# fruttasecca/approximated_personalized_pagerank

Measured on AMD Instinct MI355X. Metric: source-nodes/sec grank K=64 L=128 on RMAT-22; 1/2/4/8 MI355X + HBM GB/s, higher is better.
Workload: dtype f64

## Files before the change

approximated_personalized_pagerank_amd/csrc/merge_sv.h:

```cpp
#pragma once
#include "merge_xs.h"

namespace pprk {

constexpr int SV_R = 3;
constexpr int SV_UNIT_LOG = 31;
constexpr int SV_XS = 4;
constexpr size_t SV_LIST_BYTES = (size_t)WAVE * 12;
struct SvGeom {
  int wlog;
  int waves;
  int xt;
  int budget;
  __host__ __device__ constexpr int threads() const { return waves * WAVE; }
  __host__ __device__ constexpr int bm_words() const { return SV_R * (1 << wlog) / 64; }
  __host__ __device__ constexpr size_t sketch_bytes() const { return (size_t)SV_R * ((size_t)1 << wlog) * 4; }
  __host__ __device__ constexpr size_t p2_bytes() const { return (size_t)xt * 20 + (size_t)waves * SV_LIST_BYTES; }
  __host__ __device__ constexpr size_t region() const {
    return sketch_bytes() > p2_bytes() ? sketch_bytes() : p2_bytes();
  }
};
__host__ __device__ constexpr SvGeom sv_geom(int wlog, int waves) {
  return SvGeom{wlog, waves, SV_XS * waves * WAVE, SV_XS * waves * WAVE * 85 / 100 - waves * WAVE};
}
// ... 12 lines not shown
};
__host__ __device__ constexpr size_t x2_bytes(int T) { return (size_t)T * 20; }
__device__ __forceinline__ X2Table x2_carve(unsigned char* p, int T) {
  X2Table t;
  t.keys = reinterpret_cast<uint32_t*>(p);
  t.a = reinterpret_cast<unsigned long long*>(p + (size_t)T * 4);
  t.b = reinterpret_cast<unsigned long long*>(p + (size_t)T * 12);
  t.mask = (uint32_t)T - 1u;
  return t;
}
__device__ __forceinline__ void x2_add(const X2Table& t, int h, unsigned long long lo, uint32_t hi) {
  atomicAdd(&t.a[h], lo & 0xffffffffull);
  atomicAdd(&t.b[h], (lo >> 32) | ((unsigned long long)hi << 32));
}
__device__ __forceinline__ double x2_value(unsigned long long A, unsigned long long B, int F = XS_F) {
  const unsigned long long lo = ((B & 0xffffffffull) << 32) + A;
  const uint32_t hi = (uint32_t)(B >> 32) + (lo < A ? 1u : 0u);
  return xs_to_double(hi, lo, F);
}
__device__ __forceinline__ int x2_find(const X2Table& t, int key) {
  const uint32_t tag = (uint32_t)key + 1u;
  uint32_t g = hash32((uint32_t)key) & t.mask & ~3u;
  for (uint32_t n = 0; n <= t.mask; n += 4) {
    const uint4 q = *reinterpret_cast<const uint4*>(t.keys + g);
    const int m = xt_match(q, g, tag);
    if (m >= 0) return m;
    if (q.x == 0u || q.y == 0u || q.z == 0u || q.w == 0u) return -1;
    g = (g + 4u) & t.mask;
  }
  return -1;
}
__device__ __forceinline__ int x2_slot(const X2Table& t, int key, bool& ins) {
  const uint32_t tag = (uint32_t)key + 1u;
  uint32_t g = hash32((uint32_t)key) & t.mask & ~3u;
  ins = false;
  const uint32_t groups = (t.mask + 1u) >> 2;
  uint32_t moves = 0, races = 0;
  while (moves < groups && races <= groups) {
    const uint4 q = *reinterpret_cast<const uint4*>(t.keys + g);
    const int m = xt_match(q, g, tag);
    if (m >= 0) return m;
    const int e = q.x == 0u ? 0 : q.y == 0u ? 1 : q.z == 0u ? 2 : q.w == 0u ? 3 : -1;
    if (e >= 0) {
      const uint32_t prev = atomicCAS(&t.keys[g + e], 0u, tag);
      if (prev == 0u) { ins = true; return (int)(g + e); }
      if (prev == tag) return (int)(g + e);
      races++;
      continue;
    }
    g = (g + 4u) & t.mask;
    moves++;
  }
  return -1;
}

struct SvHash {
  uint32_t h0, h1, h2;
};
__device__ __forceinline__ SvHash sv_hash(int key) {
  const uint32_t k = (uint32_t)key;
  return SvHash{k * 0x9E3779B1u, k * 0x85EBCA77u, k * 0xC2B2AE3Du};
}
__device__ __forceinline__ uint32_t sv_units31(double p31) { return (uint32_t)p31 + 1u; }
__device__ __forceinline__ uint32_t sv_units(double p) { return sv_units31(p * 0x1p31); }
__device__ __forceinline__ uint32_t sv_thr(double theta) {
  const double x = floor(ldexp(theta, SV_UNIT_LOG) * (1.0 - 0x1p-40));
  return x <= 0.0 ? 0u : x >= 4294967295.0 ? 0xffffffffu : (uint32_t)x;
}
__device__ __forceinline__ void sv_sketch_add(uint32_t* sk, const SvHash& hs, uint32_t u, int wlog) {
  const int sh = 32 - wlog;
  atomicAdd(&sk[hs.h0 >> sh], u);
  atomicAdd(&sk[(1u << wlog) + (hs.h1 >> sh)], u);
  atomicAdd(&sk[(2u << wlog) + (hs.h2 >> sh)], u);
}
__device__ __forceinline__ bool sv_passes(const uint32_t* bm, const SvHash& hs, int wlog) {
  const int sh = 32 - wlog;
  const int rw = (1 << wlog) >> 5;
  const uint32_t w0 = bm[hs.h0 >> (sh + 5)];
  const uint32_t w1 = bm[rw + (hs.h1 >> (sh + 5))];
  const uint32_t w2 = bm[2 * rw + (hs.h2 >> (sh + 5))];
  return ((w0 >> ((hs.h0 >> sh) & 31u)) & (w1 >> ((hs.h1 >> sh) & 31u)) & (w2 >> ((hs.h2 >> sh) & 31u)) & 1u) != 0u;
}
__device__ __forceinline__ void sv_split_t(double t, unsigned long long& A, unsigned long long& B) {
  const uint32_t bh = (uint32_t)(t * 0x1p-32);
  const uint32_t bl = (uint32_t)fma(-(double)bh, 0x1p32, t);
  A = (unsigned long long)(uint32_t)(__builtin_amdgcn_fract(t) * 0x1p32);
  B = ((unsigned long long)bh << 32) | bl;
}
__device__ __forceinline__ void sv_split_add_t(unsigned long long* ab, int i, double t) {
  unsigned long long A, B;
  sv_split_t(t, A, B);
  atomicAdd(&ab[2 * i], A);
  atomicAdd(&ab[2 * i + 1], B);
}
__device__ __forceinline__ void sv_split_add(unsigned long long* ab, int i, double p) {
  sv_split_add_t(ab, i, p * 0x1p61);
}
__device__ __forceinline__ void sv_split_add_t(unsigned long long* a, unsigned long long* b, int i, double t) {
  unsigned long long A, B;
  sv_split_t(t, A, B);
  atomicAdd(&a[i], A);
  atomicAdd(&b[i], B);
}
__device__ __forceinline__ void sv_split_add(unsigned long long* a, unsigned long long* b, int i, double p) {
  sv_split_add_t(a, b, i, p * 0x1p61);
}

struct SvPt {
  uint32_t* keys;
  unsigned long long* ab;
  int* pos;
  int T;
  uint32_t gmask;
};
__host__ __device__ constexpr size_t svpt_bytes(int Lp) { return (size_t)4 * Lp * 24 + 64 * 16; }
__device__ __forceinline__ SvPt svpt_carve(unsigned char* p, int Lp) {
  SvPt t;
  t.T = 4 * Lp;
  t.ab = reinterpret_cast<unsigned long long*>(p); p += (size_t)(t.T + 64) * 16;
  t.keys = reinterpret_cast<uint32_t*>(p); p += (size_t)t.T * 4;
  t.pos = reinterpret_cast<int*>(p);
  t.gmask = (uint32_t)(t.T / 4) - 1u;
  return t;
}
constexpr uint32_t SV_OVF_BIT = 0x80000000u;
__device__ __forceinline__ uint32_t svpt_home(const SvPt& t, uint32_t h0) { return __umulhi(h0, (uint32_t)t.T) & ~3u; }
__device__ __forceinline__ int svpt_find_from(const SvPt& t, uint32_t tag, uint32_t g4) {
  for (int n = 0; n < (int)t.gmask + 1; n++) {
    g4 = (g4 + 4u) & (uint32_t)(t.T - 1);
    const uint4 q = *reinterpret_cast<const uint4*>(t.keys + g4);
    const uint32_t x = q.x & ~SV_OVF_BIT;
    if (x == tag) return (int)g4;
    if (q.y == tag) return (int)g4 + 1;
    if (q.z == tag) return (int)g4 + 2;
    if (q.w == tag) return (int)g4 + 3;
    if (x == 0u || q.y == 0u || q.z == 0u || q.w == 0u) return -1;
  }
  return -1;
}
__device__ __forceinline__ int svpt_slot(const SvPt& t, int key, uint32_t h, bool active) {
  const uint32_t tag = (uint32_t)key + 1u;
  const uint32_t g4 = svpt_home(t, h);
  const uint4 q = *reinterpret_cast<const uint4*>(t.keys + g4);
  int m = q.w == tag ? 3 : -1;
  m = q.z == tag ? 2 : m;
  m = q.y == tag ? 1 : m;
  m = (q.x & ~SV_OVF_BIT) == tag ? 0 : m;
  int slot = m >= 0 ? (int)g4 + m : -1;
  const bool more = active && m < 0 && (q.x & SV_OVF_BIT);
  if (__builtin_expect(__ballot(more) != 0ull, 0)) {
    if (more) slot = svpt_find_from(t, tag, g4);
  }
  return slot;
}

struct SvDesc {
  int32_t v;
  int32_t S;
  double factor;
  int64_t gsk;
  int64_t gpt;
  int64_t gxt;
  int32_t tg;
  int32_t pad;
};
struct SvTask { int32_t d; int32_t k; };

enum { SVM_FILL = 0, SVM_OVF = 1, SVM_U = 2, SVM_PT = 3, SVM_ROWS = 4, SVM_THETA = 8  };
__host__ __device__ constexpr size_t sv_lds_bytes(int Lp, SvGeom G) {
  return G.region() + svpt_bytes(Lp) + (size_t)G.bm_words() * 8 + 256 + 1024;
}
struct SvLds {
  unsigned char* region;
  SvPt pt;
  uint64_t* bm;
  int* misc;
  uint32_t* hist;
  int wlog;
  int bm_words;
};
__device__ __forceinline__ SvLds sv_carve(unsigned char* smem, int Lp, SvGeom G) {
  SvLds x;
  unsigned char* p = smem;
  x.region = p; p += G.region();
  x.pt = svpt_carve(p, Lp); p += svpt_bytes(Lp);
  x.bm = reinterpret_cast<uint64_t*>(p); p += (size_t)G.bm_words() * 8;
  x.misc = reinterpret_cast<int*>(p); p += 256;
  x.hist = reinterpret_cast<uint32_t*>(p);
  x.wlog = G.wlog;
  x.bm_words = G.bm_words();
  return x;
}

__device__ __forceinline__ void sv_lap(const IterArgs& a, int slot, long long& t) {
  if (!a.diag || threadIdx.x != 0) return;
  const long long now = (long long)clock64();
  diag_add(a.diag, slot, (unsigned long long)(now - t));
  t = now;
}

template <class KeyAt>
__device__ __forceinline__ void sv_build_pt_keys(const SvLds& x, int n, KeyAt keyat) {
  const SvPt& t = x.pt;
  for (int i = threadIdx.x; i < t.T; i += blockDim.x) t.keys[i] = 0u;
  for (int i = threadIdx.x; i < 2 * (t.T + 64); i += blockDim.x) t.ab[i] = 0ull;
  if (threadIdx.x < 64) x.misc[threadIdx.x] = 0;
  __syncthreads();
  for (int i = threadIdx.x; i < n; i += blockDim.x) {
    const int key = keyat(i);
    const uint32_t tag = (uint32_t)key + 1u;
    const uint32_t home = svpt_home(t, sv_hash(key).h0);
    uint32_t g4 = home;
    for (int n = 0; n <= (int)t.gmask; n++) {
      int got = -1;
#pragma unroll
      for (int j = 0; j < 4 && got < 0; j++)
        if (atomicCAS(&t.keys[g4 + j], 0u, tag) == 0u) got = (int)g4 + j;
      if (got >= 0) { t.pos[got] = i; break; }
      if (g4 == home) atomicOr(&t.keys[home], SV_OVF_BIT);
      g4 = (g4 + 4u) & (uint32_t)(t.T - 1);
    }
  }
}
__device__ __forceinline__ void sv_build_pt(const SvLds& x, const DevSlab& s, const IterArgs& a, int v, int Lp,
                                            const int32_t* seeds = nullptr) {
  const int cur = (a.active == 1) ? a.sB : a.sA;
  const int64_t r = s.row(cur, v);
  const int n = seeds ? s.L : s.len[s.lrow(cur, v)];
  sv_build_pt_keys(x, n, [&](int i) { return seeds ? (int)seeds[i] : s.key(s.ids[r + i]); });
}

template <int NS>
struct SvBatch {
  int key[2 * NS];
  double sv[2 * NS];
  int rl[NS];
  int64_t base[NS];
};
template <int NS, class G>
__device__ __forceinline__ void sv_groups(const SvBatch<NS>& bt, G g) {
  const int lane = lane_id();
#pragma unroll
  for (int k = 0; k < 2 * NS; k++) {
    const int rl = bt.rl[k >> 1];
    if ((k & 1) && rl <= WAVE) continue;
    g(k, bt.key[k], bt.sv[k], (k & 1) * WAVE + lane < rl, bt.base[k >> 1] + (k & 1) * WAVE + lane);
  }
}
__device__ __forceinline__ int64_t sv_readlane64(int64_t x, int lane) {
  const uint32_t lo = (uint32_t)__builtin_amdgcn_readlane((int)(uint32_t)x, lane);
  const uint32_t hi = (uint32_t)__builtin_amdgcn_readlane((int)(uint32_t)((uint64_t)x >> 32), lane);
  return (int64_t)(((uint64_t)hi << 32) | lo);
}
template <bool kScores, int NS, class FB, class RM = WalkNoSucc>
__device__ __forceinline__ void sv_rows(const DevGraph& g, const DevSlab& s, const IterArgs& a, int64_t c0, int64_t c1,
                                        FB fb, RM succ = RM{}) {
  const int lane = lane_id();
  const int lcl = lane < s.L ? lane : 0;
  const int lhi = WAVE + lane < s.L ? WAVE + lane : lcl;
  auto colx_at = [&](int64_t w0) { return w0 + lane < c1 ? g.colx[w0 + lane] : (int32_t)-1; };
  auto len_of = [&](int32_t cx) { return cx == -1 ? 0 : s.len[s.lrow(read_slot(a, cx), cx & 0x7fffffff)]; };
  auto base_of = [&](int32_t cx) { return cx == -1 ? (int64_t)0 : s.row(read_slot(a, cx), cx & 0x7fffffff); };
  auto rmin_of = [&](int32_t cx) {
    return cx == -1 ? 0ull : dbits(s.rmin[s.lrow(read_slot(a, cx), cx & 0x7fffffff)]);
  };
  int32_t ncx = colx_at(c0);
  int32_t nncx = c0 + WAVE < c1 ? colx_at(c0 + WAVE) : -1;
  int nln = len_of(ncx);
  unsigned long long nrm = RM::kWant ? rmin_of(ncx) : 0ull;
  for (int64_t w0 = c0; w0 < c1; w0 += WAVE) {
    const int32_t cx = ncx;
    const int ln = nln;
    if (RM::kWant) succ(ln, nrm);
    const int64_t base = base_of(cx);
    ncx = nncx;
    if (w0 + 2 * WAVE < c1) nncx = colx_at(w0 + 2 * WAVE);
    nln = len_of(ncx);
    if (RM::kWant) nrm = rmin_of(ncx);
    const int nrows = (int)min((int64_t)WAVE, c1 - w0);
    auto load = [&](int q0, SvBatch<NS>& bt) {
#pragma unroll
      for (int q = 0; q < NS; q++) {
        const bool has = q0 + q < nrows;
        const int qq = has ? q0 + q : 0;
        bt.rl[q] = has ? __builtin_amdgcn_readlane(ln, qq) : 0;
        bt.base[q] = has ? sv_readlane64(base, qq) : (int64_t)0;
        bt.key[2 * q] = s.ids[bt.base[q] + lcl];
        if (kScores) bt.sv[2 * q] = s.sc[bt.base[q] + lcl];
        const int i2 = bt.rl[q] > WAVE ? lhi : lcl;
        bt.key[2 * q + 1] = s.ids[bt.base[q] + i2];
        if (kScores) bt.sv[2 * q + 1] = s.sc[bt.base[q] + i2];
      }
    };
    auto run = [&](const SvBatch<NS>& bt) { fb(bt); };
    SvBatch<NS> ba, bb;
    load(0, ba);
    for (int q0 = 0; q0 < nrows; q0 += 2 * NS) {
      load(q0 + NS, bb);
      __builtin_amdgcn_sched_barrier(0);
      run(ba);
      __builtin_amdgcn_sched_barrier(0);
      if (q0 + NS >= nrows) break;
      load(q0 + 2 * NS, ba);
      __builtin_amdgcn_sched_barrier(0);
      run(bb);
      __builtin_amdgcn_sched_barrier(0);
    }
  }
}

__device__ __forceinline__ int64_t sv_uniform(int64_t x) {
  const uint32_t lo = (uint32_t)__builtin_amdgcn_readfirstlane((int)(uint32_t)x);
  const uint32_t hi = (uint32_t)__builtin_amdgcn_readfirstlane((int)(uint32_t)((uint64_t)x >> 32));
  return (int64_t)(((uint64_t)hi << 32) | lo);
}
__device__ __forceinline__ void sv_chunk(int64_t b0, int64_t b1, int64_t& c0, int64_t& c1) {
  const int W = blockDim.x >> 6, wv = threadIdx.x >> 6;
  const int64_t chunk = (b1 - b0 + W - 1) / W;
  c0 = sv_uniform(b0 + (int64_t)wv * chunk);
  c1 = sv_uniform(min(b1, c0 + chunk));
}

#ifndef PPR_SV_NS1
#define PPR_SV_NS1 4
#endif
#ifndef PPR_SV_NS2
#define PPR_SV_NS2 4
#endif
#ifndef PPR_SV_P2_SCORES
#define PPR_SV_P2_SCORES 0
#endif
constexpr bool SV_P2_SCORES = PPR_SV_P2_SCORES != 0;
#ifndef PPR_SV_WALK_ONLY
#define PPR_SV_WALK_ONLY 0
#endif
#ifndef PPR_SV_NO_INSERT
#define PPR_SV_NO_INSERT 0
#endif
constexpr int SV_NS1 = PPR_SV_NS1, SV_NS2 = PPR_SV_NS2;
__device__ __forceinline__ void sv_pass1(const DevGraph& g, const DevSlab& s, const IterArgs& a, const SvLds& x,
                                         int64_t b0, int64_t b1, double factor, uint32_t* sk) {
  int64_t c0, c1;
  sv_chunk(b0, b1, c0, c1);
  const double f61 = factor * 0x1p61, f31 = factor * 0x1p31;
  sv_rows<true, SV_NS1>(g, s, a, c0, c1, [&](const SvBatch<SV_NS1>& bt) {
    sv_groups(bt, [&](int, int key, double sc, bool valid, int64_t) {
      const SvHash hs = sv_hash(key);
      const int slot = svpt_slot(x.pt, key, hs.h0, valid);
      const bool inpt = valid && slot >= 0;
      if (inpt) sv_split_add_t(x.pt.ab, slot, sc * f61);
      if (valid && !inpt) sv_sketch_add(sk, hs, sv_units31(sc * f31), x.wlog);
    });
  });
}

#ifndef PPR_SV_LIST
#define PPR_SV_LIST 1
#endif
__device__ __forceinline__ void sv_insert(const SvLds& x, const X2Table& xt, const IterArgs& a, bool live, int key,
                                          double t, int budget, bool keep) {
  const int lane = lane_id();
  const bool w = live && svpt_slot(x.pt, key, sv_hash(key).h0, live) < 0;
  if (!__ballot(w)) return;
  if (a.diag && lane == 0) diag_add(a.diag, 148, 1ull);
  if (__hip_atomic_load(&x.misc[SVM_FILL], __ATOMIC_RELAXED, __HIP_MEMORY_SCOPE_WORKGROUP) > budget) {
    if (lane == 0) x.misc[SVM_OVF] = 1;
    if (keep) {
      const int hs = w ? x2_find(xt, key) : -1;
      if (hs >= 0) sv_split_add_t(xt.a, xt.b, hs, t);
    }
    return;
  }
  bool ins = false;
  int hs = -1;
  if (w) hs = x2_slot(xt, key, ins);
  const int nins = __popcll(__ballot(ins));
  if (nins && lane == 0) atomicAdd(&x.misc[SVM_FILL], nins);
  if (__ballot(w && hs < 0) && lane == 0) x.misc[SVM_OVF] = 1;
  if (hs >= 0) sv_split_add_t(xt.a, xt.b, hs, t);
  if (a.diag && lane == 0) diag_add(a.diag, 138, (unsigned long long)__popcll(__ballot(w)));
}
__device__ __forceinline__ void sv_pass2(const DevGraph& g, const DevSlab& s, const IterArgs& a, const SvLds& x,
                                         const X2Table& xt, int64_t b0, int64_t b1, double factor, int budget,
                                         bool keep = false) {
  int64_t c0, c1;
  sv_chunk(b0, b1, c0, c1);
  const uint32_t* bm32 = reinterpret_cast<const uint32_t*>(x.bm);
  const double f61 = factor * 0x1p61;
  const int lane = lane_id();
  const uint64_t lt = lanemask_lt();
  double* lst = reinterpret_cast<double*>(x.region + (size_t)(xt.mask + 1u) * 20 + (size_t)(threadIdx.x >> 6) * SV_LIST_BYTES);
  int* lsk = reinterpret_cast<int*>(lst + WAVE);
// ... 620 lines not shown
```

approximated_personalized_pagerank_amd/csrc/merge_xs.h:

```cpp
#pragma once
#include "merge_hub.h"
#include "xs_table.h"

namespace pprk {

constexpr double XR_SPEC = 0.9;

__host__ __device__ constexpr size_t lds_wave_bytes_x(int T, int Lp) {
  return (size_t)T * 16 + (size_t)Lp * 12 + 1024 + (size_t)Lp * 20;
}
__host__ __device__ constexpr size_t lds_wave_bytes_xs(int T) { return (size_t)T * 16 + 1024; }


#ifndef PPR_WX_WAVES
#define PPR_WX_WAVES 1
#endif
template <bool kSplit>
__global__ void __launch_bounds__(256, kSplit ? PPR_WX_WAVES : 1) k_merge_lds_x(DevGraph g, DevSlab s, IterArgs a, const int32_t* list,
                                                     int64_t count, int T, int Lp, unsigned long long* maxdiff,
                                                     unsigned long long* stats, int32_t* dlast, int32_t* wovl,
                                                     WList wl) {
  extern __shared__ __align__(16) unsigned char smem[];
  const int wv = threadIdx.x >> 6;
  const int64_t w = (int64_t)blockIdx.x * (blockDim.x >> 6) + wv;
  if (w >= count) return;
  unsigned char* base = smem + (size_t)wv * (kSplit ? lds_wave_bytes_xs(T) : lds_wave_bytes_x(T, Lp));
  const XTable t = xt_carve(base, T);
  uint32_t* hist = reinterpret_cast<uint32_t*>(base + (size_t)T * 16);
  uint64_t* rv = reinterpret_cast<uint64_t*>(base + (size_t)T * 16 + 1024);
  int* rk = reinterpret_cast<int*>(base + (size_t)T * 16 + 1024 + (size_t)Lp * 8);
  int* hk = reinterpret_cast<int*>(base + (size_t)T * 16 + 1024 + (size_t)Lp * 12);
  int* hv = hk + 2 * Lp;
  int* mf = hv + 2 * Lp;

  const int v = list[w];
  const int64_t b = g.rp[v], e = g.rp[v + 1];
  const double factor = merge_factor(a, e - b);
  long long tl = a.diag ? (long long)clock64() : 0;
  for (int i = lane_id(); i < T; i += WAVE) { t.keys[i] = 0u; t.lo[i] = 0ull; t.hi[i] = 0u; }
  wave_fence();
  bool bad = false;
  if (lane_id() == 0) {
    unsigned long long lo;
    uint32_t hi;
    xs_conv(self_seed(a, e - b), lo, hi, a.xsf);
    bad = xt_add(t, v, lo, hi) < 0;
  }
  wave_fence();
  unsigned long long mb = 0;
  if (a.unit) {
    unsigned long long flo;
    uint32_t fhi;
    xs_conv(factor, flo, fhi, a.xsf);
    for (int64_t e0 = b; e0 < e; e0 += WAVE) {
      const int64_t i = e0 + lane_id();
      if (i < e && xt_add(t, g.colx[i] & 0x7fffffff, flo, fhi) < 0) bad = true;
    }
  } else {
    for (int64_t e0 = b; e0 < e; e0 += WAVE)
      hub_window_walk(g, s, a, e0, min(e, e0 + WAVE), reinterpret_cast<uint8_t*>(hist),
                      [&](bool valid, int id, double sv, bool) {
                        if (valid) {
                          unsigned long long lo;
                          uint32_t hi;
                          xs_conv(sv * factor, lo, hi, a.xsf);
                          if (xt_add(t, id, lo, hi) < 0) bad = true;
                        }
                      },
                      WalkRowMin{&mb, (int)s.L});
  }
  wave_fence();
  if (__ballot(bad)) {
    if (lane_id() == 0) {
      wovl[1 + atomicAdd(&wovl[0], 1)] = v;
      if (kSplit) wl.n[w] = -1;
    }
    return;
  }
  fs_lap(a, 280, 1, tl);
#pragma unroll
  for (int o = 32; o; o >>= 1) { const unsigned long long y = __shfl_xor(mb, o); mb = y > mb ? y : mb; }
  const double tau = (!a.unit && mb) ? xs_single(bitsd(mb) * factor, a.xsf) : 0.0;
  double* vals = reinterpret_cast<double*>(t.lo);
  int* keys = reinterpret_cast<int*>(t.keys);
  double tspec = 0.0;
  if (!a.unit && !a.mc) {
    const int64_t cr = s.lrow((a.active == 1) ? a.sB : a.sA, v);
    if (s.len[cr] == s.L) tspec = fmax(tau, XR_SPEC * s.rmin[cr]);
  }
  int U = 0, D = 0, Uhi = 0;
  for (int base0 = 0; base0 < T; base0 += WAVE) {
    const int i = base0 + lane_id();
    const uint32_t kt = t.keys[i];
    const unsigned long long lo = t.lo[i];
    const bool occ = kt != 0u;
    const double x = occ ? xs_to_double(t.hi[i], lo, a.xsf) : 0.0;
    const bool keep = occ && x >= tau;
    const uint64_t m = __ballot(keep);
    D += __popcll(__ballot(occ));
    Uhi += __popcll(__ballot(keep && x >= tspec));
    wave_fence();
    if (keep) {
      const int pos = U + __popcll(m & lanemask_lt());
      vals[pos] = x;
      keys[pos] = (int)kt - 1;
    }
    wave_fence();
    U += __popcll(m);
  }
  if (tspec > tau && Uhi >= (int)s.L && Uhi < U) {
    int U2 = 0;
    for (int i0 = 0; i0 < U; i0 += WAVE) {
      const int i = i0 + lane_id();
      const double x = i < U ? vals[i] : 0.0;
      const int k = i < U ? keys[i] : 0;
      const bool keep = i < U && x >= tspec;
      const uint64_t m = __ballot(keep);
      wave_fence();
      if (keep) { const int pos = U2 + __popcll(m & lanemask_lt()); vals[pos] = x; keys[pos] = k; }
      wave_fence();
      U2 += __popcll(m);
    }
    U = U2;
  }
  if (dlast && !a.unit && lane_id() == 0) dlast[v] = D;
  fs_lap(a, 280, 2, tl);
  if (a.diag && !a.unit && lane_id() == 0) { diag_add(a.diag, 280, 1ull); diag_add(a.diag, 287, (unsigned long long)U); }
  if (kSplit) {
    wave_emit_list(wl, w, U, keys, vals, v, (int)s.L, hist);
  } else {
    finish_source(v, U, [&](int i) { return keys[i]; }, [&](int i) { return vals[i]; }, s, a, hist, rv, rk, Lp, hk, hv,
                  mf, maxdiff, stats, a.unit ? -1 : 283);
  }
}

__host__ __device__ constexpr size_t wfin_lds_bytes(int Lp) { return (size_t)Lp * 12 + 1024 + (size_t)Lp * 20; }
__global__ void __launch_bounds__(256) k_wfin(DevSlab s, IterArgs a, const int32_t* list, int64_t count, WList wl,
                                              int Lp, unsigned long long* maxdiff, unsigned long long* stats) {
  extern __shared__ __align__(16) unsigned char smem[];
  const int wv = threadIdx.x >> 6;
  const int64_t w = (int64_t)blockIdx.x * (blockDim.x >> 6) + wv;
  if (w >= count) return;
  const int n = wl.n[w];
  if (n < 0) return;
  unsigned char* base = smem + (size_t)wv * wfin_lds_bytes(Lp);
  uint64_t* rv = reinterpret_cast<uint64_t*>(base);
  int* rk = reinterpret_cast<int*>(base + (size_t)Lp * 8);
  uint32_t* hist = reinterpret_cast<uint32_t*>(base + (size_t)Lp * 12);
  int* hk = reinterpret_cast<int*>(base + (size_t)Lp * 12 + 1024);
  int* hv = hk + 2 * Lp;
  int* mf = hv + 2 * Lp;
  const int64_t o = w * (int64_t)wl.cap;
  const int32_t* lk = wl.k + o;
  const double* lv = wl.v + o;
  finish_source(list[w], n, [&](int i) { return lk[i]; }, [&](int i) { return lv[i]; }, s, a, hist, rv, rk, Lp, hk,
                hv, mf, maxdiff, stats, 283);
}

__host__ __device__ constexpr size_t xr_lds_bytes(int T, int W, int Lp) {
  return (size_t)T * 16 + (size_t)W * HUB_WALK_FLAGS + 1024 + 256 + (size_t)Lp * 32;
}

struct XDesc {
  int32_t v;
  int32_t R;
  int64_t pt_off;
  double factor, selfval;
};

enum { XM_FILL = 0, XM_OVF = 1, XM_CNT = 2, XM_U = 3, XM_MIN = 10  };

struct XrLds {
  XTable t;
  uint8_t* fl;
  WgLds w;
};

__device__ __forceinline__ XrLds xr_carve(unsigned char* smem, int T, int W, int Lp) {
  XrLds x;
  unsigned char* p = smem;
  x.t = xt_carve(p, T); p += xt_bytes(T);
  x.fl = p; p += (size_t)W * HUB_WALK_FLAGS;
  x.w = WgLds{};
  x.w.hist = reinterpret_cast<uint32_t*>(p); p += 1024;
  x.w.misc = reinterpret_cast<int*>(p); p += 256;
  x.w.rv = reinterpret_cast<uint64_t*>(p); p += (size_t)Lp * 8;
  x.w.rk = reinterpret_cast<int*>(p); p += (size_t)Lp * 4;
  x.w.hk = reinterpret_cast<int*>(p); p += (size_t)Lp * 8;
  x.w.hv = reinterpret_cast<int*>(p); p += (size_t)Lp * 8;
  x.w.mf = reinterpret_cast<int*>(p);
  return x;
}

__device__ __forceinline__ void xr_lap(const IterArgs& a, int slot, long long& t) {
  if (!a.diag || threadIdx.x != 0) return;
  const long long now = (long long)clock64();
  diag_add(a.diag, slot, (unsigned long long)(now - t));
  t = now;
}

__device__ __forceinline__ void xr_clear(const XrLds& x, int T) {
  for (int i = threadIdx.x; i < T; i += blockDim.x) { x.t.keys[i] = 0u; x.t.lo[i] = 0ull; x.t.hi[i] = 0u; }
  if (threadIdx.x < 64) x.w.misc[threadIdx.x] = 0;
}

constexpr int XR_FULL = 1 << 24;
__device__ __forceinline__ void xr_apply(const XrLds& x, bool valid, int key, double p, int budget, int F) {
  int r = 0;
  if (valid) {
    unsigned long long lo;
    uint32_t hi;
    xs_conv(p, lo, hi, F);
    r = xt_add(x.t, key, lo, hi);
  }
  const int n = __popcll(__ballot(r > 0)) + (__ballot(r < 0) ? XR_FULL : 0);
  if (n && lane_id() == 0) atomicAdd(&x.w.misc[XM_FILL], n);
}
__device__ __forceinline__ bool xr_stop(const XrLds& x, int budget) {
  return __hip_atomic_load(&x.w.misc[XM_FILL], __ATOMIC_RELAXED, __HIP_MEMORY_SCOPE_WORKGROUP) > budget;
}

constexpr int XR_SLOTS = 8;
__device__ __forceinline__ void xr_finish(const XrLds& x, int T, const DevSlab& s, const IterArgs& a,
                                          const XDesc& xd, int d, bool publish, double tau0, double tau_spec,
                                          unsigned long long* xtau, int32_t* pk, double* ps, uint32_t* pc,
                                          uint32_t* dsum, long long* tph = nullptr, int slot = 0, int cap = 0) {
  const int L = s.L;
  const int v = xd.v;
  if (publish) tau0 = fmax(tau0, bitsd(__hip_atomic_load(&xtau[d], __ATOMIC_RELAXED, __HIP_MEMORY_SCOPE_AGENT)));
  const double ts_hi = fmax(tau0, tau_spec);
  int kk[XR_SLOTS];
  double kv[XR_SLOTS];
  int c = 0, c_hi = 0;
  uint32_t kt[XR_SLOTS], kh[XR_SLOTS];
  unsigned long long kl[XR_SLOTS];
#pragma unroll
  for (int j = 0; j < XR_SLOTS; j++) {
    const int i = min(T - 1, (int)threadIdx.x + j * (int)blockDim.x);
    kt[j] = x.t.keys[i];
    kl[j] = x.t.lo[i];
    kh[j] = x.t.hi[i];
  }
#pragma unroll
  for (int j = 0; j < XR_SLOTS; j++) {
    const bool in = (int)threadIdx.x + j * (int)blockDim.x < T;
    kv[j] = xs_to_double(kh[j], kl[j], a.xsf);
    kk[j] = (in && kt[j] && kv[j] >= tau0) ? (int)kt[j] - 1 : -1;
    c += kk[j] >= 0 ? 1 : 0;
    c_hi += (kk[j] >= 0 && kv[j] >= ts_hi) ? 1 : 0;
  }
  if (tau_spec > tau0) {
    const int w_hi = wave_sum(c_hi);
    if (lane_id() == 0 && w_hi) atomicAdd(&x.w.misc[XM_CNT], w_hi);
    __syncthreads();
    if (x.w.misc[XM_CNT] >= L) {
      tau0 = ts_hi;
      c = c_hi;
#pragma unroll
      for (int j = 0; j < XR_SLOTS; j++)
        if (kk[j] >= 0 && kv[j] < ts_hi) kk[j] = -1;
    }
  }
  const int incl = wave_incl_scan(c);
  int base = 0;
  if (lane_id() == WAVE - 1 && incl) base = atomicAdd(&x.w.misc[XM_U], incl);
  base = __builtin_amdgcn_readlane(base, WAVE - 1) + incl - c;
  __syncthreads();
  int* dk = reinterpret_cast<int*>(x.t.keys);
  double* dv = reinterpret_cast<double*>(x.t.lo);
#pragma unroll
  for (int j = 0; j < XR_SLOTS; j++)
    if (kk[j] >= 0) { dk[base] = kk[j]; dv[base] = kv[j]; base++; }
  __syncthreads();
  const int D = x.w.misc[XM_FILL];
  const int U = x.w.misc[XM_U];
  if (threadIdx.x == 0 && D) atomicAdd(&dsum[d], (uint32_t)D);
  const uint32_t ts = tie_salt(v);
  auto keyat = [&](int i) { return dk[i]; };
  auto valat = [&](int i) { return dv[i]; };
  SelCrit sc;
  sc.tie = false; sc.pa = 0; sc.ma = 0; sc.pb = 0; sc.mb = 0;
  const bool cut = U > L && !(cap && !publish && U <= cap);
  if (tph) xr_lap(a, slot, *tph);
  if (cut) sc = wg_select_top(x.w, U, L, keyat, valat, [](int) { return true; }, ts);
  if (tph) xr_lap(a, slot + 1, *tph);
  double tb = tau0;
  if (publish) {
    if (cut) {
      unsigned long long* wmin = reinterpret_cast<unsigned long long*>(&x.w.misc[XM_MIN]);
      if (threadIdx.x == 0) *wmin = ~0ull;
      __syncthreads();
      unsigned long long mn = ~0ull;
      for (int i = threadIdx.x; i < U; i += blockDim.x) {
        const unsigned long long vb = dbits(dv[i]);
        if (sel_test(sc, vb, tie_w(dk[i], ts))) mn = vb < mn ? vb : mn;
      }
      mn = wave_min_u64(mn);
      if (lane_id() == 0 && mn != ~0ull) atomicMin(wmin, mn);
      __syncthreads();
      if (threadIdx.x == 0 && *wmin != ~0ull) atomicMax(&xtau[d], *wmin);
      __syncthreads();
    }
    tb = fmax(tb, bitsd(__hip_atomic_load(&xtau[d], __ATOMIC_RELAXED, __HIP_MEMORY_SCOPE_AGENT)));
  }
  for (int i0 = 0; i0 < U; i0 += blockDim.x) {
    const int i = i0 + threadIdx.x;
    bool k = false;
    if (i < U) {
      const uint64_t vb = dbits(dv[i]);
      k = dv[i] >= tb && (!cut || sel_test(sc, vb, tie_w(dk[i], ts)));
    }
    const uint64_t m = __ballot(k);
    uint32_t b0 = 0;
    if (m && lane_id() == 0) b0 = atomicAdd(&pc[d], (uint32_t)__popcll(m));
    b0 = (uint32_t)__shfl((int)b0, 0);
    if (k) {
      const int64_t o = xd.pt_off + b0 + __popcll(m & lanemask_lt());
      pk[o] = dk[i];
      ps[o] = dv[i];
    }
  }
  if (tph) xr_lap(a, slot + 2, *tph);
}

__host__ __device__ constexpr size_t xf1_lds_bytes(int Lp) { return (size_t)Lp * 12 + 1024 + (size_t)Lp * 20; }
__global__ void __launch_bounds__(64) k_xfin1(DevSlab s, IterArgs a, const XDesc* xdesc, int d0, const int32_t* pk,
                                              const double* ps, const uint32_t* pc, const uint32_t* dsum,
                                              const int32_t* skip, int32_t* dlast, int Lp,
                                              unsigned long long* maxdiff, unsigned long long* stats) {
  extern __shared__ __align__(16) unsigned char smem[];
  const int d = d0 + (int)blockIdx.x;
  if (skip[d]) return;
  const XDesc xd = xdesc[d];
  uint64_t* rv = reinterpret_cast<uint64_t*>(smem);
  int* rk = reinterpret_cast<int*>(smem + (size_t)Lp * 8);
  uint32_t* hist = reinterpret_cast<uint32_t*>(smem + (size_t)Lp * 12);
  int* hk = reinterpret_cast<int*>(smem + (size_t)Lp * 12 + 1024);
  int* hv = hk + 2 * Lp;
  int* mf = hv + 2 * Lp;
  const int n = (int)pc[d];
  if (dlast && !a.unit && lane_id() == 0) dlast[xd.v] = (int32_t)dsum[d];
  const int32_t* lk = pk + xd.pt_off;
  const double* lv = ps + xd.pt_off;
  finish_source(xd.v, n, [&](int i) { return lk[i]; }, [&](int i) { return lv[i]; }, s, a, hist, rv, rk, Lp, hk, hv, mf,
                maxdiff, stats);
}

__device__ __forceinline__ bool xr_in(int key, int r, int R) {
  return R == 1 || (int)(((uint64_t)hash_b((uint32_t)key) * (uint32_t)R) >> 32) == r;
}

struct XTask { int32_t d; int32_t r; };

__global__ void __launch_bounds__(1024) k_xr(DevGraph g, DevSlab s, IterArgs a, const XDesc* xdesc,
                                             const XTask* tasks, int T, int budget, int Lp, unsigned long long* xtau,
                                             int32_t* pk, double* ps, uint32_t* pc, uint32_t* dsum,
                                             int32_t* oflag, int32_t* ovl, int xcap) {
  extern __shared__ __align__(16) unsigned char smem[];
  const int W = blockDim.x >> 6, wv = threadIdx.x >> 6;
  const XrLds x = xr_carve(smem, T, W, Lp);
  const XTask tk = tasks[blockIdx.x];
  const XDesc xd = xdesc[tk.d];
  const int v = xd.v, R = xd.R, r = tk.r;
  long long tph = a.diag ? (long long)clock64() : 0;
  xr_clear(x, T);
  __syncthreads();
  if (threadIdx.x == 0 && xr_in(v, r, R)) {
    unsigned long long lo;
    uint32_t hi;
    xs_conv(xd.selfval, lo, hi, a.xsf);
    xt_add(x.t, v, lo, hi);
    x.w.misc[XM_FILL] = 1;
  }
  __syncthreads();
  xr_lap(a, 183, tph);
  const int64_t b = g.rp[v], e = g.rp[v + 1];
  const double factor = xd.factor;
  unsigned long long mb = 0;
  uint8_t* fl = x.fl + (size_t)wv * HUB_WALK_FLAGS;
  auto fn = [&](bool valid, int id, double sv, bool) {
#if defined(PPR_XR_WALK_ONLY)
    if (valid && id == -9 && sv == -1.0) x.w.misc[XM_FILL] = 1;
    return;
#endif
    if (xr_stop(x, budget)) return;
    xr_apply(x, valid && xr_in(id, r, R), id, sv * factor, budget, a.xsf);
  };
  if (a.unit) {
    for (int64_t e0 = b + (int64_t)wv * WAVE; e0 < e; e0 += (int64_t)W * WAVE) {
      const int64_t i = e0 + lane_id();
      const int key = i < e ? (g.colx[i] & 0x7fffffff) : 0;
      if (xr_stop(x, budget)) break;
      xr_apply(x, i < e && xr_in(key, r, R), key, factor, budget, a.xsf);
    }
  } else {
    const int64_t chunk = (e - b + W - 1) / W;
    const int64_t c0 = b + (int64_t)wv * chunk, c1 = min(e, c0 + chunk);
    for (int64_t w0 = c0; w0 < c1; w0 += WAVE)
      hub_window_walk(g, s, a, w0, min(c1, w0 + WAVE), fl, fn, WalkRowMin{&mb, (int)s.L});
  }
  __syncthreads();
  xr_lap(a, 184, tph);
  if (a.diag && threadIdx.x == 0) {
    diag_add(a.diag, 182, 1ull);
    diag_add(a.diag, 188, (unsigned long long)(xd.R > 0 ? (e - b) : 0));
    diag_add(a.diag, 189, (unsigned long long)x.w.misc[XM_FILL]);
  }
  if (x.w.misc[XM_FILL] > budget) {
    if (threadIdx.x == 0 && atomicExch(&oflag[tk.d], 1) == 0) ovl[1 + atomicAdd(&ovl[0], 1)] = tk.d;
    return;
  }
#pragma unroll
  for (int o = 32; o; o >>= 1) { const unsigned long long y = __shfl_xor(mb, o); mb = y > mb ? y : mb; }
  if (lane_id() == 0 && mb) atomicMax(reinterpret_cast<unsigned long long*>(&x.w.misc[8]), mb);
  __syncthreads();
  const unsigned long long mbb = *reinterpret_cast<unsigned long long*>(&x.w.misc[8]);
  const double tau_rows = (!a.unit && mbb) ? xs_single(bitsd(mbb) * factor, a.xsf) : 0.0;
  double tau_spec = 0.0;
  if (R == 1 && !a.unit && !a.mc) {
    const int64_t cr = s.lrow((a.active == 1) ? a.sB : a.sA, v);
    if (s.len[cr] == s.L) tau_spec = XR_SPEC * s.rmin[cr];
  }
  xr_finish(x, T, s, a, xd, tk.d, R > 1, tau_rows, tau_spec, xtau, pk, ps, pc, dsum, a.diag ? &tph : nullptr, 185, xcap);
}

constexpr int XB_BATCH = 4;
__global__ void __launch_bounds__(1024) k_xb(DevSlab s, IterArgs a, const HubDesc* desc, const HubTask* tasks,
                                             const int32_t* cm, const uint32_t* staged, const HubRec* st,
                                             const unsigned long long* tau_b, int T, int budget, int Lp,
                                             unsigned long long* xtau, int32_t* pk, double* ps, uint32_t* pc,
                                             uint32_t* dsum, int32_t* oflag, int32_t* ovl, const int64_t* rp) {
  extern __shared__ __align__(16) unsigned char smem[];
  const int W = blockDim.x >> 6, wv = threadIdx.x >> 6;
  const XrLds x = xr_carve(smem, T, W, Lp);
  const HubTask tk = tasks[blockIdx.x];
  const HubDesc d = desc[tk.d];
  int64_t start, nb;
  hub_bucket_range(d, cm, staged[tk.d], tk.x, start, nb);
  const int v = d.v;
  const int64_t deg = rp[v + 1] - rp[v];
  const double factor = merge_factor(a, deg);
  long long tph = a.diag ? (long long)clock64() : 0;
  xr_clear(x, T);
  __syncthreads();
  if (threadIdx.x == 0 && (int)hub_digit(v, d.logP) == tk.x) {
    unsigned long long lo;
    uint32_t hi;
    xs_conv(self_seed(a, deg), lo, hi, a.xsf);
    xt_add(x.t, v, lo, hi);
    x.w.misc[XM_FILL] = 1;
  }
  __syncthreads();
  const HubRec* rec = st + start;
  const int64_t ng = (nb + WAVE - 1) / WAVE;
  struct Batch { HubRec r[XB_BATCH]; };
  auto load = [&](int64_t g0, Batch& hr) {
#pragma unroll
    for (int k = 0; k < XB_BATCH; k++) {
      const int64_t q = (g0 + (int64_t)k * W) * WAVE + lane_id();
      hr.r[k] = rec[q < nb ? q : nb - 1];
    }
  };
  int hk = -1;
  unsigned long long hlo = 0ull;
  uint32_t hhi = 0u;
  auto apply = [&](int64_t g0, const Batch& hr) {
    bool v[XB_BATCH];
    int key[XB_BATCH];
    unsigned long long lo[XB_BATCH];
    uint32_t hi[XB_BATCH], g[XB_BATCH];
    uint4 q[XB_BATCH];
#pragma unroll
    for (int k = 0; k < XB_BATCH; k++) {
      const int64_t gk = g0 + (int64_t)k * W;
      key[k] = rec_key(hr.r[k]);
      v[k] = gk < ng && gk * WAVE + lane_id() < nb;
      xs_conv(rec_sc(hr.r[k]) * factor, lo[k], hi[k], a.xsf);
      if (v[k] && key[k] == hk) {
        const unsigned long long nl = hlo + lo[k];
        hhi += hi[k] + (nl < hlo ? 1u : 0u);
        hlo = nl;
        v[k] = false;
      }
      g[k] = hash32((uint32_t)key[k]) & x.t.mask & ~3u;
    }
#pragma unroll
    for (int k = 0; k < XB_BATCH; k++) q[k] = *reinterpret_cast<const uint4*>(x.t.keys + g[k]);
    int h[XB_BATCH];
#pragma unroll
    for (int k = 0; k < XB_BATCH; k++) {
      h[k] = xt_match(q[k], g[k], (uint32_t)key[k] + 1u);
      if (__ballot(v[k] && h[k] < 0)) {
        if (xr_stop(x, budget)) {
          if (h[k] < 0) v[k] = false;
        } else {
          bool ins = false;
          if (v[k] && h[k] < 0) h[k] = xt_slot(x.t, key[k], ins);
          const bool full = v[k] && h[k] < 0;
          if (full) v[k] = false;
          const int nins = __popcll(__ballot(ins)) + (__ballot(full) ? XR_FULL : 0);
          if (nins && lane_id() == 0) atomicAdd(&x.w.misc[XM_FILL], nins);
        }
      }
    }
    unsigned long long old[XB_BATCH];
#pragma unroll
    for (int k = 0; k < XB_BATCH; k++) {
      if (!v[k]) { h[k] = 0; lo[k] = 0ull; hi[k] = 0u; }
      old[k] = atomicAdd(&x.t.lo[h[k]], lo[k]);
    }
#pragma unroll
    for (int k = 0; k < XB_BATCH; k++) atomicAdd(&x.t.hi[h[k]], hi[k] + ((old[k] + lo[k] < old[k]) ? 1u : 0u));
  };
  Batch ba, bb;
  const int64_t step = (int64_t)W * XB_BATCH;
  if (wv < ng) {
    load(wv, ba);
    const bool v0 = (int64_t)wv * WAVE + lane_id() < nb;
    const int k0 = rec_key(ba.r[0]);
    int best = 0;
#pragma unroll
    for (int c = 0; c < 8; c++) {
      const int cand = __builtin_amdgcn_readlane(k0, c * 8);
      const int n = __popcll(__ballot(v0 && k0 == cand));
      if (n > best && __builtin_amdgcn_readlane((int)v0, c * 8)) { best = n; hk = cand; }
    }
    if (best < 8) hk = -1;
  }
  for (int64_t g0 = wv; g0 < ng; g0 += 2 * step) {
    load(g0 + step < ng ? g0 + step : g0, bb);
    __builtin_amdgcn_sched_barrier(0);
    apply(g0, ba);
    __builtin_amdgcn_sched_barrier(0);
    if (g0 + step >= ng) break;
    load(g0 + 2 * step < ng ? g0 + 2 * step : g0, ba);
    __builtin_amdgcn_sched_barrier(0);
    apply(g0 + step, bb);
    __builtin_amdgcn_sched_barrier(0);
  }
  if (hk >= 0 && (hlo | hhi)) {
    const int r = xt_add(x.t, hk, hlo, hhi);
    if (r) atomicAdd(&x.w.misc[XM_FILL], r > 0 ? 1 : XR_FULL);
  }
  __syncthreads();
  xr_lap(a, 155, tph);
  if (a.diag && threadIdx.x == 0) {
    diag_add(a.diag, 154, 1ull);
    diag_add(a.diag, 159, (unsigned long long)nb);
  }
  if (x.w.misc[XM_FILL] > budget) {
    if (threadIdx.x == 0 && atomicExch(&oflag[tk.d], 1) == 0) ovl[1 + atomicAdd(&ovl[0], 1)] = v;
    return;
  }
  const double tau_rows = (!a.unit && tau_b[tk.d]) ? xs_single(bitsd(tau_b[tk.d]) * factor, a.xsf) : 0.0;
  XDesc xd;
  xd.v = v; xd.R = 0; xd.pt_off = d.pt_off; xd.factor = factor; xd.selfval = 0.0;
  xr_finish(x, T, s, a, xd, tk.d, true, tau_rows, 0.0, xtau, pk, ps, pc, dsum, a.diag ? &tph : nullptr, 156);
}

constexpr int XF_STAGE = 4096;
// ... 74 lines not shown
```

approximated_personalized_pagerank_amd/csrc/xs_table.h:

```cpp
#pragma once
#include "ppr_common.h"

namespace pprk {

__device__ __forceinline__ void xs_conv(double p, unsigned long long& lo, uint32_t& hi, int F = XS_F) {
  const unsigned long long b = dbits(p);
  int e = (int)((b >> 52) & 0x7ffu);
  unsigned long long m = b & ((1ull << 52) - 1ull);
  if (e) m |= 1ull << 52; else e = 1;
  const int sh = e - 1075 + F;
  if (sh >= 0) {
    lo = m << sh;
    hi = sh > 11 ? (uint32_t)(m >> (64 - sh)) : 0u;
  } else {
    lo = -sh < 64 ? (m >> -sh) : 0ull;
    hi = 0u;
  }
}

__device__ __forceinline__ double xs_to_double(uint32_t hi, unsigned long long lo, int F = XS_F) {
  if (hi == 0u) return ldexp((double)lo, -F);
  const int n = 32 - __clz(hi);
  const unsigned long long top = ((unsigned long long)hi << (64 - n)) | (lo >> n);
  const unsigned long long sticky = (lo & ((1ull << n) - 1ull)) != 0ull ? 1ull : 0ull;
  return ldexp((double)(top | sticky), n - F);
}

__device__ __forceinline__ double xs_single(double p, int F = XS_F) {
  unsigned long long lo;
  uint32_t hi;
  xs_conv(p, lo, hi, F);
  return xs_to_double(hi, lo, F);
}

struct XTable {
  uint32_t* keys;
  unsigned long long* lo;
  uint32_t* hi;
  uint32_t mask;
};

__device__ __forceinline__ int xt_add(const XTable& t, int key, unsigned long long xlo, uint32_t xhi) {
  const uint32_t tag = (uint32_t)key + 1u;
  uint32_t g = hash32((uint32_t)key) & t.mask & ~3u;
  int ins = 0;
  uint32_t h = 0;
  const uint32_t groups = (t.mask + 1u) >> 2;
  uint32_t moves = 0, races = 0;
  for (;;) {
    if (moves >= groups || races > groups) return -1;
    const uint4 q = *reinterpret_cast<const uint4*>(t.keys + g);
    if (q.x == tag) { h = g; break; }
    if (q.y == tag) { h = g + 1; break; }
    if (q.z == tag) { h = g + 2; break; }
    if (q.w == tag) { h = g + 3; break; }
    const int e = q.x == 0u ? 0 : q.y == 0u ? 1 : q.z == 0u ? 2 : q.w == 0u ? 3 : -1;
    if (e >= 0) {
      const uint32_t prev = atomicCAS(&t.keys[g + e], 0u, tag);
      if (prev == 0u) { h = g + e; ins = 1; break; }
      if (prev == tag) { h = g + e; break; }
      races++;
      continue;
    }
    g = (g + 4u) & t.mask;
    moves++;
  }
  const unsigned long long old = atomicAdd(&t.lo[h], xlo);
  const uint32_t up = xhi + ((old + xlo < old) ? 1u : 0u);
  if (up) atomicAdd(&t.hi[h], up);
  return ins;
}

__device__ __forceinline__ int xt_match(const uint4& q, uint32_t g, uint32_t tag) {
  return q.x == tag ? (int)g : q.y == tag ? (int)g + 1 : q.z == tag ? (int)g + 2 : q.w == tag ? (int)g + 3 : -1;
}
__device__ __forceinline__ int xt_slot(const XTable& t, int key, bool& ins) {
  const uint32_t tag = (uint32_t)key + 1u;
  uint32_t g = hash32((uint32_t)key) & t.mask & ~3u;
  ins = false;
  const uint32_t groups = (t.mask + 1u) >> 2;
  uint32_t moves = 0, races = 0;
  while (moves < groups && races <= groups) {
    const uint4 q = *reinterpret_cast<const uint4*>(t.keys + g);
    const int m = xt_match(q, g, tag);
    if (m >= 0) return m;
    const int e = q.x == 0u ? 0 : q.y == 0u ? 1 : q.z == 0u ? 2 : q.w == 0u ? 3 : -1;
    if (e >= 0) {
      const uint32_t prev = atomicCAS(&t.keys[g + e], 0u, tag);
      if (prev == 0u) { ins = true; return (int)(g + e); }
      if (prev == tag) return (int)(g + e);
      races++;
      continue;
    }
    g = (g + 4u) & t.mask;
    moves++;
  }
  return -1;
}

__host__ __device__ constexpr size_t xt_bytes(int T) { return (size_t)T * 16; }
// ... 11 lines not shown
```

Before: 3.977 million.

## Use FP-arithmetic fixed-point conversion and batched row walk in LDS merge

Replaces the bit-manipulation double-to-fixed-point conversion (exponent/mantissa shifts with branches) with a branch-free floating-point split into three 32-bit words, and pre-multiplies the scale into the factor once per row. It also moves the batched, software-pipelined row walker into a shared header and uses it in the LDS merge kernel for short rows (L <= 128) in place of the per-window hub walk. The FP-based conversion truncates instead of shifting mantissa bits, which can change rounding or behaviour for very large or very small values.

```diff
diff --git a/approximated_personalized_pagerank_amd/csrc/merge_sv.h b/approximated_personalized_pagerank_amd/csrc/merge_sv.h
--- a/approximated_personalized_pagerank_amd/csrc/merge_sv.h
+++ b/approximated_personalized_pagerank_amd/csrc/merge_sv.h
@@ -118,10 +118,9 @@
   return ((w0 >> ((hs.h0 >> sh) & 31u)) & (w1 >> ((hs.h1 >> sh) & 31u)) & (w2 >> ((hs.h2 >> sh) & 31u)) & 1u) != 0u;
 }
 __device__ __forceinline__ void sv_split_t(double t, unsigned long long& A, unsigned long long& B) {
-  const uint32_t bh = (uint32_t)(t * 0x1p-32);
-  const uint32_t bl = (uint32_t)fma(-(double)bh, 0x1p32, t);
-  A = (unsigned long long)(uint32_t)(__builtin_amdgcn_fract(t) * 0x1p32);
-  B = ((unsigned long long)bh << 32) | bl;
+  const XsWords w = xs_words(t);
+  A = (unsigned long long)w.a;
+  B = ((unsigned long long)w.bh << 32) | w.bl;
 }
 __device__ __forceinline__ void sv_split_add_t(unsigned long long* ab, int i, double t) {
   unsigned long long A, B;
@@ -266,84 +265,6 @@
   sv_build_pt_keys(x, n, [&](int i) { return seeds ? (int)seeds[i] : s.key(s.ids[r + i]); });
 }
 
-template <int NS>
-struct SvBatch {
-  int key[2 * NS];
-  double sv[2 * NS];
-  int rl[NS];
-  int64_t base[NS];
-};
-template <int NS, class G>
-__device__ __forceinline__ void sv_groups(const SvBatch<NS>& bt, G g) {
-  const int lane = lane_id();
-#pragma unroll
-  for (int k = 0; k < 2 * NS; k++) {
-    const int rl = bt.rl[k >> 1];
-    if ((k & 1) && rl <= WAVE) continue;
-    g(k, bt.key[k], bt.sv[k], (k & 1) * WAVE + lane < rl, bt.base[k >> 1] + (k & 1) * WAVE + lane);
-  }
-}
-__device__ __forceinline__ int64_t sv_readlane64(int64_t x, int lane) {
-  const uint32_t lo = (uint32_t)__builtin_amdgcn_readlane((int)(uint32_t)x, lane);
-  const uint32_t hi = (uint32_t)__builtin_amdgcn_readlane((int)(uint32_t)((uint64_t)x >> 32), lane);
-  return (int64_t)(((uint64_t)hi << 32) | lo);
-}
-template <bool kScores, int NS, class FB, class RM = WalkNoSucc>
-__device__ __forceinline__ void sv_rows(const DevGraph& g, const DevSlab& s, const IterArgs& a, int64_t c0, int64_t c1,
-                                        FB fb, RM succ = RM{}) {
-  const int lane = lane_id();
-  const int lcl = lane < s.L ? lane : 0;
-  const int lhi = WAVE + lane < s.L ? WAVE + lane : lcl;
-  auto colx_at = [&](int64_t w0) { return w0 + lane < c1 ? g.colx[w0 + lane] : (int32_t)-1; };
-  auto len_of = [&](int32_t cx) { return cx == -1 ? 0 : s.len[s.lrow(read_slot(a, cx), cx & 0x7fffffff)]; };
-  auto base_of = [&](int32_t cx) { return cx == -1 ? (int64_t)0 : s.row(read_slot(a, cx), cx & 0x7fffffff); };
-  auto rmin_of = [&](int32_t cx) {
-    return cx == -1 ? 0ull : dbits(s.rmin[s.lrow(read_slot(a, cx), cx & 0x7fffffff)]);
-  };
-  int32_t ncx = colx_at(c0);
-  int32_t nncx = c0 + WAVE < c1 ? colx_at(c0 + WAVE) : -1;
-  int nln = len_of(ncx);
-  unsigned long long nrm = RM::kWant ? rmin_of(ncx) : 0ull;
-  for (int64_t w0 = c0; w0 < c1; w0 += WAVE) {
-    const int32_t cx = ncx;
-    const int ln = nln;
-    if (RM::kWant) succ(ln, nrm);
-    const int64_t base = base_of(cx);
-    ncx = nncx;
-    if (w0 + 2 * WAVE < c1) nncx = colx_at(w0 + 2 * WAVE);
-    nln = len_of(ncx);
-    if (RM::kWant) nrm = rmin_of(ncx);
-    const int nrows = (int)min((int64_t)WAVE, c1 - w0);
-    auto load = [&](int q0, SvBatch<NS>& bt) {
-#pragma unroll
-      for (int q = 0; q < NS; q++) {
-        const bool has = q0 + q < nrows;
-        const int qq = has ? q0 + q : 0;
-        bt.rl[q] = has ? __builtin_amdgcn_readlane(ln, qq) : 0;
-        bt.base[q] = has ? sv_readlane64(base, qq) : (int64_t)0;
-        bt.key[2 * q] = s.ids[bt.base[q] + lcl];
-        if (kScores) bt.sv[2 * q] = s.sc[bt.base[q] + lcl];
-        const int i2 = bt.rl[q] > WAVE ? lhi : lcl;
-        bt.key[2 * q + 1] = s.ids[bt.base[q] + i2];
-        if (kScores) bt.sv[2 * q + 1] = s.sc[bt.base[q] + i2];
-      }
-    };
-    auto run = [&](const SvBatch<NS>& bt) { fb(bt); };
-    SvBatch<NS> ba, bb;
-    load(0, ba);
-    for (int q0 = 0; q0 < nrows; q0 += 2 * NS) {
-      load(q0 + NS, bb);
-      __builtin_amdgcn_sched_barrier(0);
-      run(ba);
-      __builtin_amdgcn_sched_barrier(0);
-      if (q0 + NS >= nrows) break;
-      load(q0 + 2 * NS, ba);
-      __builtin_amdgcn_sched_barrier(0);
-      run(bb);
-      __builtin_amdgcn_sched_barrier(0);
-    }
-  }
-}
 
 __device__ __forceinline__ int64_t sv_uniform(int64_t x) {
   const uint32_t lo = (uint32_t)__builtin_amdgcn_readfirstlane((int)(uint32_t)x);
diff --git a/approximated_personalized_pagerank_amd/csrc/merge_xs.h b/approximated_personalized_pagerank_amd/csrc/merge_xs.h
--- a/approximated_personalized_pagerank_amd/csrc/merge_xs.h
+++ b/approximated_personalized_pagerank_amd/csrc/merge_xs.h
@@ -1,5 +1,6 @@
 #pragma once
 #include "merge_hub.h"
+#include "walk_rows.h"
 #include "xs_table.h"
 
 namespace pprk {
@@ -15,6 +16,10 @@
 #ifndef PPR_WX_WAVES
 #define PPR_WX_WAVES 1
 #endif
+#ifndef PPR_WX_NS
+#define PPR_WX_NS 4
+#endif
+constexpr int WX_NS = PPR_WX_NS;
 template <bool kSplit>
 __global__ void __launch_bounds__(256, kSplit ? PPR_WX_WAVES : 1) k_merge_lds_x(DevGraph g, DevSlab s, IterArgs a, const int32_t* list,
                                                      int64_t count, int T, int Lp, unsigned long long* maxdiff,
@@ -48,6 +53,7 @@
   }
   wave_fence();
   unsigned long long mb = 0;
+  const double ft = factor * xs_scale(a.xsf);
   if (a.unit) {
     unsigned long long flo;
     uint32_t fhi;
@@ -56,6 +62,17 @@
       const int64_t i = e0 + lane_id();
       if (i < e && xt_add(t, g.colx[i] & 0x7fffffff, flo, fhi) < 0) bad = true;
     }
+  } else if (s.L <= 2 * WAVE) {
+    sv_rows<true, WX_NS>(g, s, a, b, e, [&](const SvBatch<WX_NS>& bt) {
+      sv_groups(bt, [&](int, int id, double sv, bool valid, int64_t) {
+        if (valid) {
+          unsigned long long lo;
+          uint32_t hi;
+          xs_conv_t(sv * ft, lo, hi);
+          if (xt_add(t, id, lo, hi) < 0) bad = true;
+        }
+      });
+    }, WalkRowMin{&mb, (int)s.L});
   } else {
     for (int64_t e0 = b; e0 < e; e0 += WAVE)
       hub_window_walk(g, s, a, e0, min(e, e0 + WAVE), reinterpret_cast<uint8_t*>(hist),
@@ -63,7 +80,7 @@
                         if (valid) {
                           unsigned long long lo;
                           uint32_t hi;
-                          xs_conv(sv * factor, lo, hi, a.xsf);
+                          xs_conv_t(sv * ft, lo, hi);
                           if (xt_add(t, id, lo, hi) < 0) bad = true;
                         }
                       },
@@ -205,12 +222,12 @@
 }
 
 constexpr int XR_FULL = 1 << 24;
-__device__ __forceinline__ void xr_apply(const XrLds& x, bool valid, int key, double p, int budget, int F) {
+__device__ __forceinline__ void xr_apply(const XrLds& x, bool valid, int key, double t, int budget) {
   int r = 0;
   if (valid) {
     unsigned long long lo;
     uint32_t hi;
-    xs_conv(p, lo, hi, F);
+    xs_conv_t(t, lo, hi);
     r = xt_add(x.t, key, lo, hi);
   }
   const int n = __popcll(__ballot(r > 0)) + (__ballot(r < 0) ? XR_FULL : 0);
@@ -376,6 +393,7 @@
   xr_lap(a, 183, tph);
   const int64_t b = g.rp[v], e = g.rp[v + 1];
   const double factor = xd.factor;
+  const double ft = factor * xs_scale(a.xsf);
   unsigned long long mb = 0;
   uint8_t* fl = x.fl + (size_t)wv * HUB_WALK_FLAGS;
   auto fn = [&](bool valid, int id, double sv, bool) {
@@ -384,14 +402,14 @@
     return;
 #endif
     if (xr_stop(x, budget)) return;
-    xr_apply(x, valid && xr_in(id, r, R), id, sv * factor, budget, a.xsf);
+    xr_apply(x, valid && xr_in(id, r, R), id, sv * ft, budget);
   };
   if (a.unit) {
     for (int64_t e0 = b + (int64_t)wv * WAVE; e0 < e; e0 += (int64_t)W * WAVE) {
       const int64_t i = e0 + lane_id();
       const int key = i < e ? (g.colx[i] & 0x7fffffff) : 0;
       if (xr_stop(x, budget)) break;
-      xr_apply(x, i < e && xr_in(key, r, R), key, factor, budget, a.xsf);
+      xr_apply(x, i < e && xr_in(key, r, R), key, ft, budget);
     }
   } else {
     const int64_t chunk = (e - b + W - 1) / W;
@@ -440,6 +458,7 @@
   const int v = d.v;
   const int64_t deg = rp[v + 1] - rp[v];
   const double factor = merge_factor(a, deg);
+  const double ft = factor * xs_scale(a.xsf);
   long long tph = a.diag ? (long long)clock64() : 0;
   xr_clear(x, T);
   __syncthreads();
@@ -475,7 +494,7 @@
       const int64_t gk = g0 + (int64_t)k * W;
       key[k] = rec_key(hr.r[k]);
       v[k] = gk < ng && gk * WAVE + lane_id() < nb;
-      xs_conv(rec_sc(hr.r[k]) * factor, lo[k], hi[k], a.xsf);
+      xs_conv_t(rec_sc(hr.r[k]) * ft, lo[k], hi[k]);
       if (v[k] && key[k] == hk) {
         const unsigned long long nl = hlo + lo[k];
         hhi += hi[k] + (nl < hlo ? 1u : 0u);
diff --git a/approximated_personalized_pagerank_amd/csrc/walk_rows.h b/approximated_personalized_pagerank_amd/csrc/walk_rows.h
--- /dev/null
+++ b/approximated_personalized_pagerank_amd/csrc/walk_rows.h
@@ -0,0 +1,85 @@
+#pragma once
+#include "merge_wave.h"
+
+namespace pprk {
+
+template <int NS>
+struct SvBatch {
+  int key[2 * NS];
+  double sv[2 * NS];
+  int rl[NS];
+  int64_t base[NS];
+};
+template <int NS, class G>
+__device__ __forceinline__ void sv_groups(const SvBatch<NS>& bt, G g) {
+  const int lane = lane_id();
+#pragma unroll
+  for (int k = 0; k < 2 * NS; k++) {
+    const int rl = bt.rl[k >> 1];
+    if ((k & 1) && rl <= WAVE) continue;
+    g(k, bt.key[k], bt.sv[k], (k & 1) * WAVE + lane < rl, bt.base[k >> 1] + (k & 1) * WAVE + lane);
+  }
+}
+__device__ __forceinline__ int64_t sv_readlane64(int64_t x, int lane) {
+  const uint32_t lo = (uint32_t)__builtin_amdgcn_readlane((int)(uint32_t)x, lane);
+  const uint32_t hi = (uint32_t)__builtin_amdgcn_readlane((int)(uint32_t)((uint64_t)x >> 32), lane);
+  return (int64_t)(((uint64_t)hi << 32) | lo);
+}
+template <bool kScores, int NS, class FB, class RM = WalkNoSucc>
+__device__ __forceinline__ void sv_rows(const DevGraph& g, const DevSlab& s, const IterArgs& a, int64_t c0, int64_t c1,
+                                        FB fb, RM succ = RM{}) {
+  const int lane = lane_id();
+  const int lcl = lane < s.L ? lane : 0;
+  const int lhi = WAVE + lane < s.L ? WAVE + lane : lcl;
+  auto colx_at = [&](int64_t w0) { return w0 + lane < c1 ? g.colx[w0 + lane] : (int32_t)-1; };
+  auto len_of = [&](int32_t cx) { return cx == -1 ? 0 : s.len[s.lrow(read_slot(a, cx), cx & 0x7fffffff)]; };
+  auto base_of = [&](int32_t cx) { return cx == -1 ? (int64_t)0 : s.row(read_slot(a, cx), cx & 0x7fffffff); };
+  auto rmin_of = [&](int32_t cx) {
+    return cx == -1 ? 0ull : dbits(s.rmin[s.lrow(read_slot(a, cx), cx & 0x7fffffff)]);
+  };
+  int32_t ncx = colx_at(c0);
+  int32_t nncx = c0 + WAVE < c1 ? colx_at(c0 + WAVE) : -1;
+  int nln = len_of(ncx);
+  unsigned long long nrm = RM::kWant ? rmin_of(ncx) : 0ull;
+  for (int64_t w0 = c0; w0 < c1; w0 += WAVE) {
+    const int32_t cx = ncx;
+    const int ln = nln;
+    if (RM::kWant) succ(ln, nrm);
+    const int64_t base = base_of(cx);
+    ncx = nncx;
+    if (w0 + 2 * WAVE < c1) nncx = colx_at(w0 + 2 * WAVE);
+    nln = len_of(ncx);
+    if (RM::kWant) nrm = rmin_of(ncx);
+    const int nrows = (int)min((int64_t)WAVE, c1 - w0);
+    auto load = [&](int q0, SvBatch<NS>& bt) {
+#pragma unroll
+      for (int q = 0; q < NS; q++) {
+        const bool has = q0 + q < nrows;
+        const int qq = has ? q0 + q : 0;
+        bt.rl[q] = has ? __builtin_amdgcn_readlane(ln, qq) : 0;
+        bt.base[q] = has ? sv_readlane64(base, qq) : (int64_t)0;
+        bt.key[2 * q] = s.ids[bt.base[q] + lcl];
+        if (kScores) bt.sv[2 * q] = s.sc[bt.base[q] + lcl];
+        const int i2 = bt.rl[q] > WAVE ? lhi : lcl;
+        bt.key[2 * q + 1] = s.ids[bt.base[q] + i2];
+        if (kScores) bt.sv[2 * q + 1] = s.sc[bt.base[q] + i2];
+      }
+    };
+    auto run = [&](const SvBatch<NS>& bt) { fb(bt); };
+    SvBatch<NS> ba, bb;
+    load(0, ba);
+    for (int q0 = 0; q0 < nrows; q0 += 2 * NS) {
+      load(q0 + NS, bb);
+      __builtin_amdgcn_sched_barrier(0);
+      run(ba);
+      __builtin_amdgcn_sched_barrier(0);
+      if (q0 + NS >= nrows) break;
+      load(q0 + 2 * NS, ba);
+      __builtin_amdgcn_sched_barrier(0);
+      run(bb);
+      __builtin_amdgcn_sched_barrier(0);
+    }
+  }
+}
+
+}
diff --git a/approximated_personalized_pagerank_amd/csrc/xs_fixed.h b/approximated_personalized_pagerank_amd/csrc/xs_fixed.h
--- /dev/null
+++ b/approximated_personalized_pagerank_amd/csrc/xs_fixed.h
@@ -0,0 +1,46 @@
+#pragma once
+#include <cmath>
+#include <cstdint>
+
+#if defined(__HIPCC__)
+#define XSF_HD __host__ __device__ inline __attribute__((always_inline))
+#else
+#define XSF_HD inline
+#endif
+
+namespace pprk {
+
+XSF_HD double xs_pow2(int e) { return __builtin_bit_cast(double, (uint64_t)(1023 + e) << 52); }
+XSF_HD double xs_scale(int F) { return xs_pow2(F - 32); }
+
+XSF_HD double xs_fract(double t) {
+#if defined(__HIP_DEVICE_COMPILE__)
+  return __builtin_amdgcn_fract(t);
+#else
+  return t - std::floor(t);
+#endif
+}
+
+struct XsWords {
+  uint32_t a;
+  uint32_t bl;
+  uint32_t bh;
+};
+XSF_HD XsWords xs_words(double t) {
+  XsWords w;
+  w.bh = (uint32_t)(t * 0x1p-32);
+  w.bl = (uint32_t)__builtin_fma(-(double)w.bh, 0x1p32, t);
+  w.a = (uint32_t)(xs_fract(t) * 0x1p32);
+  return w;
+}
+
+XSF_HD void xs_conv_t(double t, unsigned long long& lo, uint32_t& hi) {
+  const XsWords w = xs_words(t);
+  lo = ((unsigned long long)w.bl << 32) | w.a;
+  hi = w.bh;
+}
+XSF_HD void xs_conv_f(double p, unsigned long long& lo, uint32_t& hi, int F) {
+  xs_conv_t(p * xs_scale(F), lo, hi);
+}
+
+}
diff --git a/approximated_personalized_pagerank_amd/csrc/xs_table.h b/approximated_personalized_pagerank_amd/csrc/xs_table.h
--- a/approximated_personalized_pagerank_amd/csrc/xs_table.h
+++ b/approximated_personalized_pagerank_amd/csrc/xs_table.h
@@ -1,21 +1,11 @@
 #pragma once
 #include "ppr_common.h"
+#include "xs_fixed.h"
 
 namespace pprk {
 
 __device__ __forceinline__ void xs_conv(double p, unsigned long long& lo, uint32_t& hi, int F = XS_F) {
-  const unsigned long long b = dbits(p);
-  int e = (int)((b >> 52) & 0x7ffu);
-  unsigned long long m = b & ((1ull << 52) - 1ull);
-  if (e) m |= 1ull << 52; else e = 1;
-  const int sh = e - 1075 + F;
-  if (sh >= 0) {
-    lo = m << sh;
-    hi = sh > 11 ? (uint32_t)(m >> (64 - sh)) : 0u;
-  } else {
-    lo = -sh < 64 ? (m >> -sh) : 0ull;
-    hi = 0u;
-  }
+  xs_conv_f(p, lo, hi, F);
 }
 
 __device__ __forceinline__ double xs_to_double(uint32_t hi, unsigned long long lo, int F = XS_F) {
```

Result: faster. 4.050 million, median of 6 (+1.8%).
